# MarvelMathesh/sincformer-metacog-speech-enhancement

Hardware: AMD Instinct MI355X
Metric: audio frames/sec/GPU (16 kHz, 512-frame utts) + mask RMSE vs CPU ref (higher is better)
Workload: dtype fp16 MFMA operands (PerceptionAgent, fusion, Conformer GEMMs, heads) + bf16 attention core, fp32 accumulate (ops.POLICIES['mixed']); 1 GPU; B256 x 512-frame utterances (L40880, T512) forward; batch_per_gpu=256, samples=40880, frames_per_utt=512, launch=eager launches, streams=2, precision_policy=mixed

## Files before the change

include/sincformer_hip.h:

```cpp
#ifndef SINCFORMER_HIP_H
#define SINCFORMER_HIP_H
#ifdef __cplusplus
extern "C" {
#endif

#define SFM_OK 0
#define SFM_ERR_ARG (-1)
#define SFM_ERR_SHAPE (-2)
#define SFM_ERR_LAUNCH (-3)
#define SFM_DT_BF16 0
#define SFM_DT_F16 1

#define SFM_EPI_NONE 0
#define SFM_EPI_SWISH 1
#define SFM_EPI_GELU 2
#define SFM_EPI_RESID 3
#define SFM_EPI_GLU 4
#define SFM_EPI_SIGMOID 5
#define SFM_EPI_TANH_SCALE 6
#define SFM_EPI_SIGMA 7
#define SFM_EPI_CPEA 8

#define SFM_LAYERNORM_MAX_D 512
#define SFM_ATTN_QTILE 128
// ... 201 lines not shown
                      int act, int dtype, float* ws, void* stream);
long long sfm_gn_bwd_reduce_ws_floats(int B, int L, int C);
int sfm_gn_bwd_coefs(float* S, const float* gamma1, const float* rstd1, const float* gamma2, const float* rstd2,
                     float* coef1, float* coef2, float* dparam, int B, int L, int C, int G, void* stream);
int sfm_gn_bwd_apply(const void* dout, int dout_f32, const void* x1, int x1_f32, const float* sc1, const float* sh1,
                     const float* mean1, const float* rstd1, const float* coef1, void* dx1, int dx1_f32, const void* x2,
                     int x2_f32, const float* sc2, const float* sh2, const float* mean2, const float* rstd2,
                     const float* coef2, void* dx2, int dx2_f32, int B, int L, int C, int G, int act, int dtype,
                     void* stream);
int sfm_maa_update_stats(const float* sigma, long long n, double* acc, float* stats, long long* num_updates, float momentum,
                         void* stream);
int sfm_maa_forward(const float* sigma, const float* stats, const float* params, float* logits, float* probs,
                    long long* decisions, float* confidence, long long n, void* stream);
int sfm_maa_backward(const float* sigma, const float* stats, const float* params, const float* g_logits, const float* g_probs,
                     const float* g_conf, float* dsigma, void* H1, void* H2, void* dZ1, void* dZ2, void* GL, void* XN,
                     long long n, int dtype, void* stream);
int sfm_vq_forward(const float* x, const float* centroids, int M, float* q, long long* idx, double* acc, long long n,
                   void* stream);
int sfm_vq_backward(const float* x, const long long* idx, const float* centroids, int M, const float* g_q,
                    const float* g_loss, float beta, float* dx, float* dcent, long long n, void* stream);
long long sfm_sumsq_ws_doubles(long long n);
int sfm_sumsq(const float* g, long long n, double* out, double* ws, void* stream);
int sfm_adamw_step(float* p, float* g, float* m, float* v, long long n, double* ctl, float lr, float beta1, float beta2,
                   float eps, float wd, float inv_scale, float max_norm, int write_back_grad, void* stream);
int sfm_adamw_step_masked(float* p, float* g, float* m, float* v, long long n, double* ctl, float lr, float beta1, float beta2,
                          float eps, float wd, float inv_scale, float max_norm, int write_back_grad, const long long* spans,
                          const float* touched, int n_params, void* stream);
int sfm_adamw_step_scaled(float* p, float* g, float* m, float* v, long long n, double* ctl, float lr, float beta1, float beta2,
                          float eps, float wd, float inv_world, float max_norm, int write_back_grad, const long long* spans,
                          const float* touched, int n_params, float* loss_scale, float growth_factor, float backoff_factor,
                          int growth_interval, void* stream);
long long sfm_tn_ws_floats(int M, int N, int K);
int sfm_gemm16_tn(const void* G, const void* X, float* dW, float* db, int M, int N, int K, int ldg, int ldx, int ldw,
                  int dtype, float* ws, long long ws_floats, void* stream);
int sfm_conv_wgrad16(const void* G, const void* x, float* dW, float* db, int B, int Lout, int Lin, int Cin, int N, int ksize,
                     int stride, int pad, long long x_batch_stride, int ldg, int ldw, int dtype, float* ws, long long ws_floats,
                     void* stream);
long long sfm_colsum_ws_floats(int M, int N);
int sfm_colsum(const void* G, float* out, int M, int N, int ldg, int g_f32, int dtype, float* ws, void* stream);
long long sfm_layernorm_bwd_ws_floats(int M, int D);
int sfm_layernorm_bwd(const float* x, const float* gamma, const float* dy, const float* dres, float* dx,
                      float* dgamma, float* dbeta, int M, int D, int ldx, int ld, float eps, float* ws, void* stream);
int sfm_layernorm_bwd_ex(const float* x, const float* gamma, const void* dy, int dy_16, const float* dres, float* dx,
                         float* dgamma, float* dbeta, int M, int D, int ldx, int ldy, int ld, float eps, int dtype,
                         float* ws, void* stream);
int sfm_layernorm_bwd_next(const float* x, const float* gamma, const void* dy, int dy_16, const float* dres, float* dx,
                           float* dgamma, float* dbeta, int M, int D, int ldx, int ldy, int ld, float eps, int dtype,
                           void* next16, float next_alpha, float next_p, unsigned int next_seed, float* ws, void* stream);
int sfm_ew_train(const void* z, const void* g, void* out, long long M, int N, int mode, int g_f32, int out_f32,
                 float alpha, float p, unsigned int seed, int dtype, void* stream);
long long sfm_col_stats_ws_floats(int M, int C);
int sfm_col_stats(const float* y, const float* aux, const float* mean, const float* rstd, float* S, int M, int C, float* ws,
                  void* stream);
int sfm_col_pilot(const float* y, float* K, int M, int C, void* stream);
int sfm_col_stats_shifted(const float* y, const float* K, float* S, int M, int C, float* ws, void* stream);
int sfm_add_cols(const float* a, const float* b, float* out, long long M, int C, int Cb, long long lda, long long ldb, long long ldo,
                 void* stream);
int sfm_lstm_hprev16(const float* h, void* out, int B, int T, int H, int dtype, void* stream);
int sfm_bn_finalize(const float* S, const float* K, const float* gamma, const float* beta, float* run_mean, float* run_var,
                    float* mean, float* rstd, float* sc, float* sh, int C, long long M, float eps, float momentum, int eval_mode,
                    void* stream);
int sfm_bn_swish_bwd(const void* g, const float* y, const float* mean, const float* rstd, const float* gamma,
                     const float* beta, float* S, float* dy, int M, int C, int g_f32, int pass, int dtype,
                     float* ws, void* stream);
long long sfm_dwconv_wgrad_scratch_floats(int B, int T, int C, int KS);
int sfm_dwconv_wgrad(const void* x, const float* dy, float* dw, float* db, float* scratch, int B, int T, int C, int KS,
                     int dtype, void* stream);
int sfm_attention_fwd_train(const void* qkv, void* out, float* lse, int B, int T, int H, int hd, int ldqkv,
                            int ldo, int koff, int voff, long long qkv_batch_stride, long long o_batch_stride,
                            float scale, float p_drop, unsigned int seed, int dtype, void* stream);
int sfm_attention_bwd(const void* qkv, const void* O, const void* dO, const float* lse, float* delta, void* dqkv,
                      int B, int T, int H, int hd, int ldqkv, int ldo, int koff, int voff, float p_drop,
                      unsigned int seed, int dtype, void* stream);
int sfm_lin256(const void* A, const void* W, const float* bias, void* out, int M, int NW, int lda, int ldo, int glu, int dtype,
               int out_dtype, void* stream);
int sfm_ln_lin256(const float* X32, int ldx, const float* lnw, const float* lnb, float eps, const void* W, const float* bias,
                  void* out, int M, int NW, int ldo, int glu, int dtype, int out_dtype, void* stream);
int sfm_headpool_frames_per_tile(int Tin, int Tout);
int sfm_headpool(const void* xd, const void* W, const float* bias, void* pooled, float* gn_partial, int B, int Tin, int Tout, int NW,
                 int lda, int ldp, int gcols, int dtype, void* stream);

int sfm_bilstm_layer(const float* xg, const float* whh, float* out, int B, int T, int H, int dtype, void* stream);
int sfm_bilstm_layer_ex(const float* xg, const float* whh, float* out, int B, int T, int H, int w16, void* stream);
int sfm_bilstm_layer_train_ex(const float* xg, const float* whh, float* out, float* save, int B, int T, int H, int w16, void* stream);
int sfm_bilstm_layer_train(const float* xg, const float* whh, float* out, float* save, int B, int T, int H, int dtype,
                           void* stream);
int sfm_bilstm_layer_bwd(const float* save, const float* whh, const float* dout, float* dxg, int B, int T, int H,
                         void* stream);
int sfm_memory_fwd(const float* emb, const float* params, float* bias_out, float* gate_out, int* top_idx,
                   float* sim_out, int B, int key_dim, int value_dim, int slots, float temperature, void* stream);
long long sfm_memory_param_floats(int key_dim, int value_dim, int slots);
long long sfm_memory_bwd_ws_floats(int B, int key_dim, int value_dim, int slots);
int sfm_memory_bwd(const float* emb, const float* params, const float* d_out, const float* d_gate, float* d_emb,
                   float* dparams, int B, int key_dim, int value_dim, int slots, float temperature, float* ws, void* stream);

long long sfm_pstoi_loss_ws_doubles(int B, int T, int frame_len);
int sfm_pstoi_loss(const float* e0, const float* e1, const float* c0, const float* c1, const float* band_w, float* loss,
                   float* g0, float* g1, double* ws, int B, int T, int F, int NB, int frame_len, float beta_db, int layout,
                   void* stream);
long long sfm_mse_loss_ws_doubles(long long n);
int sfm_mse_loss(const float* pred, const float* target, float* loss, float* grad, double* ws, long long n, void* stream);

int sfm_adv_sn_fwd(const long long* table, int n_layers, void* packed, void* packed_lo, float* saved, int training, float eps,
                   int dtype, void* stream);
int sfm_adv_sn_bwd(const float* G, const float* W, const float* u, const float* v, const float* sigma, float* dW,
                   const float* db_in, float* db, const float* g, float cnorm, int N, int Cin, int ksize, int Cp, int accumulate,
                   void* stream);
int sfm_adv_stage(const float* x, const float* im, void* x16, void* x16lo, float* x32, int B, int F, int T, int Cp, int pair,
                  int dtype, void* stream);
int sfm_adv_stage_bwd(const float* d, const float* re, const float* im, float* dx, float* dx_im, const float* g, float cnorm, int B,
                      int F, int T, int Cp, int pair, void* stream);
long long sfm_adv_leaky_ws_doubles(long long n);
int sfm_adv_leaky(const float* z, const float* z_real, void* a16, void* a16lo, double* ws, double* loss, float scale, long long n,
                  int dtype, void* stream);
int sfm_adv_leaky_bwd(const float* incoming, const float* z, const float* z_real, const float* g, float w_fm, float cnorm,
                      void* dz16, long long n, int dtype, void* stream);
int sfm_adv_pool(const float* in32, float* out32, void* out16, void* out16lo, int B, int Tin, int F, int Cp, int dtype,
                 void* stream);
int sfm_adv_pool_bwd(const float* dnext, float* dx, int B, int Tin, int Cp, void* stream);
long long sfm_adv_head_ws_doubles(int B, int T);
int sfm_adv_head(const void* a16, const void* a16lo, const void* w16, const void* w16lo, const float* bias, float* out, double* ws,
                 double* loss, float target, float scale, int B, int T, int C, int dtype, void* stream);
long long sfm_adv_head_bwd_ws_floats(int B, int T, int C);
int sfm_adv_head_bwd(const void* a16, const void* w16, const float* out, const float* g, float coef, float cnorm, float target,
                     float* da, float* dwb, float* ws, int B, int T, int C, int dtype, void* stream);

int sfm_mask_irm(const float* clean_mag, const float* noise_mag, float* out, long long n, float p, float eps, void* stream);
int sfm_mask_corr(const float* noisy, const float* clean, const float* noise, float* rho_s, float* rho_n, long long n, float eps,
                  void* stream);
int sfm_mask_pcirm(const float* clean_mag, const float* noise_mag, const float* rho_s, const float* rho_n, const float* phi1,
                   const float* phi2, float* out, long long n, float eps, void* stream);
int sfm_mask_quantize(const float* pcirm, const double* table, float* out, long long n, int M, void* stream);
long long sfm_mix_scale_ws_doubles(int B, int L);
int sfm_mix_scale(const float* clean, const float* bank, const int* bank_off, const int* noise_ids, const float* snr_db,
                  const int* lengths, double* ws, float* scale, int B, int L, int n_noise, void* stream);
int sfm_mix_apply(const float* clean, const float* bank, const int* bank_off, const int* noise_ids, const int* lengths,
                  const float* scale, float* noisy, float* noise_rows, int B, int L, int n_noise, void* stream);
int sfm_curriculum_mask(const float* cr, const float* ci, const float* nr, const float* ni, const float* scale,
                        const double* table, float* yr, float* yi, float* mask, int B, int T, int F, int kind, float p, float eps,
                        int M, void* stream);

int sfm_pso_frame_coef(const float* pcirm, const double* table, double* a, double* b, int B, int C, int T, int M, void* stream);
long long sfm_pso_split_ws_doubles(int B, int Lmax);
int sfm_pso_split(const float* noisy, const float* clean, const int* lengths, const int* samp_off, const double* a,
                  const double* b, float* ya, float* yb, float* clean_packed, double* ws, double* S, int B, int Lmax, int T,
                  int frame, int hop, void* stream);
int sfm_pso_fitness(const float* cr, const float* ci, const float* ar, const float* ai, const float* br, const float* bi,
                    const int* frame_off, const int* lengths, const double* S, const double* pos, const int* stopped,
                    double* partial, int B, int N, int F, int NC, void* stream);
int sfm_pso_step(const double* partial, const double* fitness, const int* frame_off, const double* draws, const double* params,
                 double* pos, double* vel, double* pbest_pos, double* pbest_fit, double* gbest, double* hist, int* iters,
                 int* stopped, int B, int N, int NC, int it, int max_iter, int maximize, void* stream);
int sfm_pso_quantize(const float* pcirm, const double* table, const double* middle, float* out, int B, long long CT, int M,
                     void* stream);

int sfm_gammatone_fir(const float* sig, const float* taps, const int* lengths, float* out, int B, int L, int C, int K, void* stream);
int sfm_gammatone_tf_fits(int K, int hop);
int sfm_gammatone_tf(const float* sig, const float* taps, const float* tw, const int* lengths, float* partial, int B, int L, int C,
                     int K, int hop, int nblocks, void* stream);
int sfm_gammatone_moments(const float* y, const float* tw, const int* lengths, float* partial, int B, int L, int C, int T, int w,
                          int frame, int hop, void* stream);
int sfm_gammatone_tf_finish(const float* partial, const float* rot, const int* lengths, float* mag, float* phase, float* re,
                            float* im, int B, int C, int T, int P, int two, int L, int frame, int hop, int N, void* stream);

int sfm_haircell(const float* x, const double* par, double* out, int N, int L, void* stream);
int sfm_haircell_frames(const float* x, const double* par, const int* lengths, double* frames, int N, int C, int L, int frame,
// ... 31 lines not shown
```

sincformer_metacog_speech_enhancement_amd/csrc/lstm.hip:

```cpp
#include "sfm_common.h"

constexpr int LSTM_FWD_LPU = 4;

#define DPP_XOR1 0xB1
#define DPP_XOR2 0x4E
#define DPP_HALF_MIRROR 0x141
#define DPP_Q0 0x00
#define DPP_Q1 0x55
#define DPP_Q2 0xAA
#define DPP_Q3 0xFF

__device__ __forceinline__ float fast_sigmoid(float x) {
  return __builtin_amdgcn_rcpf(1.0f + __builtin_amdgcn_exp2f(-1.44269504088896340736f * x));
}

template <int H, int LPU>
__global__ __launch_bounds__(LPU * H) void bilstm_layer_kernel(const float* __restrict__ xg,
                                                               const float* __restrict__ whh,
                                                               float* __restrict__ out, int T, float* __restrict__ save) {
  constexpr int KS = H / LPU;
  constexpr int SL = KS + 4;
  __shared__ __attribute__((aligned(16))) float hs[2][LPU * SL];
  const int tid = threadIdx.x;
  const int j = tid / LPU, ks = tid % LPU;
  const int dir = blockIdx.x, b = blockIdx.y;
  float w[4][KS];
#pragma unroll
  for (int g = 0; g < 4; ++g) {
    const float* wr = whh + ((long long)dir * 4 * H + g * H + j) * H + ks * KS;
#pragma unroll
    for (int i = 0; i < KS; ++i) w[g][i] = wr[i];
  }
  if (tid < LPU * SL) { hs[0][tid] = 0.f; hs[1][tid] = 0.f; }
  __syncthreads();
  float c = 0.f;
  const int mygate = ks & 3;
  const float* xb = xg + (long long)b * T * (8 * H) + (long long)dir * 4 * H + mygate * H + j;
  float* ob = out + (long long)b * T * (2 * H) + dir * H + j;
  int t = dir ? (T - 1) : 0;
  const int dt = dir ? -1 : 1;
  const float gsc = (mygate == 2) ? 2.0f : 1.0f, gof = (mygate == 2) ? -1.0f : 0.0f;
  const int hslot = (j / KS) * SL + (j % KS);
  float xnext = xb[(long long)t * (8 * H)];
  for (int s = 0; s < T; ++s, t += dt) {
    const float xcur = xnext;
    if (s + 1 < T) xnext = xb[(long long)(t + dt) * (8 * H)];
    const float* hc = hs[s & 1] + ks * SL;
    float a[4] = {0.f, 0.f, 0.f, 0.f};
#pragma unroll
    for (int i = 0; i < KS; i += 4) {
      const f32x4 hv = *reinterpret_cast<const f32x4*>(hc + i);
#pragma unroll
      for (int g = 0; g < 4; ++g) {
        a[g] += w[g][i] * hv[0];
        a[g] += w[g][i + 1] * hv[1];
        a[g] += w[g][i + 2] * hv[2];
        a[g] += w[g][i + 3] * hv[3];
      }
    }
#pragma unroll
    for (int g = 0; g < 4; ++g) {
      a[g] = dpp_perm_add<DPP_XOR1>(a[g]);
      a[g] = dpp_perm_add<DPP_XOR2>(a[g]);
      if (LPU == 8) a[g] = dpp_perm_add<DPP_HALF_MIRROR>(a[g]);
    }
    const float pre = ((mygate == 0) ? a[0] : (mygate == 1) ? a[1] : (mygate == 2) ? a[2] : a[3]) + xcur;
    const float act = gsc * fast_sigmoid(gsc * pre) + gof;
    const float ig = dpp_perm<DPP_Q0>(act), fg = dpp_perm<DPP_Q1>(act);
    const float cg = dpp_perm<DPP_Q2>(act), og = dpp_perm<DPP_Q3>(act);
    c = fg * c + ig * cg;
    const float h = og * (2.0f * fast_sigmoid(2.0f * c) - 1.0f);
    if (ks == 0) {
      hs[(s + 1) & 1][hslot] = h;
      ob[(long long)t * (2 * H)] = h;
    }
    if (save) {
      float* sv = save + ((((long long)b * T + t) * 2 + dir) * 5) * H + j;
      if (ks < 4) sv[mygate * H] = act;
      if (ks == LPU - 4) sv[4 * H] = c;
    }
    asm volatile("s_waitcnt lgkmcnt(0)\n\ts_barrier" ::: "memory");
  }
}

typedef _Float16 lstm_h2 __attribute__((ext_vector_type(2)));
template <int H, int LPU, bool SAVE>
__global__ __launch_bounds__(LPU * H, 4) void bilstm_layer16_kernel(const float* __restrict__ xg, const float* __restrict__ whh,
                                                                    float* __restrict__ out, int T, float* __restrict__ save) {
  constexpr int KS = H / LPU;
  constexpr int KW = KS / 2;
  constexpr int SLW = KW + 4;
  static_assert(KW % 4 == 0, "16-byte slice reads");
  __shared__ __attribute__((aligned(16))) uint32_t hs[2][LPU * SLW];
  const int tid = threadIdx.x;
  const int j = tid / LPU, ks = tid % LPU;
  const int dir = blockIdx.x, b = blockIdx.y;
  lstm_h2 w[4][KW];
#pragma unroll
  for (int g = 0; g < 4; ++g) {
    const float* wr = whh + ((long long)dir * 4 * H + g * H + j) * H + ks * KS;
#pragma unroll
    for (int i = 0; i < KW; ++i) w[g][i] = lstm_h2{(_Float16)wr[2 * i], (_Float16)wr[2 * i + 1]};
    __builtin_amdgcn_sched_barrier(0);
  }
  if (tid < LPU * SLW) { hs[0][tid] = 0u; hs[1][tid] = 0u; }
  __syncthreads();
  float c = 0.f;
  const int mygate = ks & 3;
  const float* xb = xg + (long long)b * T * (8 * H) + (long long)dir * 4 * H + mygate * H + j;
  float* ob = out + (long long)b * T * (2 * H) + dir * H + j;
  int t = dir ? (T - 1) : 0;
  const int dt = dir ? -1 : 1;
  const float gsc = (mygate == 2) ? 2.0f : 1.0f, gof = (mygate == 2) ? -1.0f : 0.0f;
  const uint32_t hbase = (uint32_t)(uintptr_t)(lds_ptr_t)&hs[0][0];
  const uint32_t hslot = hbase + ((j / KS) * SLW * 2 + (j % KS)) * 2;
  const uint32_t hread = hbase + ks * SLW * 4;
  float xnext = xb[(long long)t * (8 * H)];
  for (int s = 0; s < T; ++s, t += dt) {
    const float xcur = xnext;
    if (s + 1 < T) xnext = xb[(long long)(t + dt) * (8 * H)];
    const uint32_t hc = hread + (uint32_t)((s & 1) * LPU * SLW * 4);
    float a[4] = {0.f, 0.f, 0.f, 0.f};
    u32x4 hv[KW / 4];
#pragma unroll
    for (int q = 0; q < KW / 4; ++q) asm volatile("ds_read_b128 %0, %1 offset:%2" : "=v"(hv[q]) : "v"(hc), "n"(q * 16) : "memory");
    if constexpr (KW / 4 == 4) {
      asm volatile("s_waitcnt lgkmcnt(2)" : "+v"(hv[0]), "+v"(hv[1])::"memory");
      asm volatile("s_waitcnt lgkmcnt(0)" : "+v"(hv[2]), "+v"(hv[3])::"memory");
    } else {
      static_assert(KW / 4 == 2, "H 128 or 64 with 4 lanes per unit");
      asm volatile("s_waitcnt lgkmcnt(0)" : "+v"(hv[0]), "+v"(hv[1])::"memory");
    }
#pragma unroll
    for (int q = 0; q < KW / 4; ++q) {
#pragma unroll
      for (int e = 0; e < 4; ++e) {
        const uint32_t hd = hv[q][e];
        const lstm_h2 hp = __builtin_bit_cast(lstm_h2, hd);
#pragma unroll
        for (int g = 0; g < 4; ++g) a[g] = __builtin_amdgcn_fdot2(w[g][4 * q + e], hp, a[g], false);
      }
    }
#pragma unroll
    for (int g = 0; g < 4; ++g) {
      a[g] = dpp_perm_add<DPP_XOR1>(a[g]);
      a[g] = dpp_perm_add<DPP_XOR2>(a[g]);
      if (LPU == 8) a[g] = dpp_perm_add<DPP_HALF_MIRROR>(a[g]);
    }
    const float pre = ((mygate == 0) ? a[0] : (mygate == 1) ? a[1] : (mygate == 2) ? a[2] : a[3]) + xcur;
    const float act = gsc * fast_sigmoid(gsc * pre) + gof;
    const float ig = dpp_perm<DPP_Q0>(act), fg = dpp_perm<DPP_Q1>(act);
    const float cg = dpp_perm<DPP_Q2>(act), og = dpp_perm<DPP_Q3>(act);
    c = fg * c + ig * cg;
    const float h = og * (2.0f * fast_sigmoid(2.0f * c) - 1.0f);
    if (ks == 0) {
      const uint32_t hb = (uint32_t)__builtin_bit_cast(unsigned short, (_Float16)h);
      asm volatile("ds_write_b16 %0, %1" ::"v"(hslot + (uint32_t)(((s + 1) & 1) * LPU * SLW * 4)), "v"(hb) : "memory");
      ob[(long long)t * (2 * H)] = h;
    }
    if (SAVE) {
      float* sv = save + ((((long long)b * T + t) * 2 + dir) * 5) * H + j;
      if (ks < 4) sv[mygate * H] = act;
      if (ks == LPU - 4) sv[4 * H] = c;
    }
    asm volatile("s_waitcnt lgkmcnt(0)\n\ts_barrier" ::: "memory");
  }
}

template <int H, int LPU>
__global__ __launch_bounds__(LPU * H) void bilstm_layer_bwd_kernel(const float* __restrict__ save,
                                                                 const float* __restrict__ whh,
                                                                 const float* __restrict__ dout,
                                                                 float* __restrict__ dxg, int T) {
  constexpr int G4 = 4 * H;
  constexpr int KS = G4 / LPU;
  constexpr int SL = KS + 4;
  __shared__ __attribute__((aligned(16))) float das[2][LPU * SL];
  const int tid = threadIdx.x;
  const int j = tid / LPU, ks = tid % LPU;
  const int dir = blockIdx.x, b = blockIdx.y;
  float w[KS];
#pragma unroll
  for (int i = 0; i < KS; ++i) w[i] = whh[((long long)dir * G4 + ks * KS + i) * H + j];
  for (int i = tid; i < LPU * SL; i += LPU * H) { das[0][i] = 0.f; das[1][i] = 0.f; }
  __syncthreads();
  const long long cb = (long long)b * T;
  float dh_rec = 0.f, dc_next = 0.f;
  const int dt = dir ? -1 : 1;
  int t = dir ? 0 : (T - 1);
  float nx[7] = {0.f, 0.f, 0.f, 0.f, 0.f, 0.f, 0.f};
  auto fetch = [&](int tt) {
    const float* sv = save + (((cb + tt) * 2 + dir) * 5) * H + j;
    nx[0] = sv[0]; nx[1] = sv[H]; nx[2] = sv[2 * H]; nx[3] = sv[3 * H]; nx[4] = sv[4 * H];
    const int tp = tt - dt;
    nx[5] = (tp >= 0 && tp < T) ? save[(((cb + tp) * 2 + dir) * 5 + 4) * H + j] : 0.f;
    nx[6] = dout[(cb + tt) * (2 * H) + dir * H + j];
  };
  if (ks == 0) fetch(t);
  for (int s = 0; s < T; ++s, t -= dt) {
    if (ks == 0) {
      const float ig = nx[0], fg = nx[1], gg = nx[2], og = nx[3], c = nx[4], cp = nx[5];
      const float dh = nx[6] + dh_rec;
      if (s + 1 < T) fetch(t - dt);
      const float tc = 2.0f * fast_sigmoid(2.0f * c) - 1.0f;
      const float dc = dh * og * (1.0f - tc * tc) + dc_next;
      const float dai = dc * gg * ig * (1.0f - ig);
      const float daf = dc * cp * fg * (1.0f - fg);
      const float dag = dc * ig * (1.0f - gg * gg);
      const float dao = dh * tc * og * (1.0f - og);
      dc_next = dc * fg;
      float* dx = dxg + (cb + t) * (8 * H) + (long long)dir * G4 + j;
      dx[0] = dai; dx[H] = daf; dx[2 * H] = dag; dx[3 * H] = dao;
      float* da = das[s & 1];
      da[((0 * H + j) / KS) * SL + (0 * H + j) % KS] = dai;
      da[((1 * H + j) / KS) * SL + (1 * H + j) % KS] = daf;
      da[((2 * H + j) / KS) * SL + (2 * H + j) % KS] = dag;
      da[((3 * H + j) / KS) * SL + (3 * H + j) % KS] = dao;
    }
    asm volatile("s_waitcnt lgkmcnt(0)\n\ts_barrier" ::: "memory");
    const float* dc_ = das[s & 1] + ks * SL;
    float a = 0.f, a2 = 0.f;
#pragma unroll
    for (int i = 0; i < KS; i += 8) {
      const f32x4 v = *reinterpret_cast<const f32x4*>(dc_ + i);
      const f32x4 u = *reinterpret_cast<const f32x4*>(dc_ + i + 4);
      a += w[i] * v[0];
      a2 += w[i + 4] * u[0];
      a += w[i + 1] * v[1];
      a2 += w[i + 5] * u[1];
      a += w[i + 2] * v[2];
      a2 += w[i + 6] * u[2];
      a += w[i + 3] * v[3];
      a2 += w[i + 7] * u[3];
    }
    a += a2;
    a = dpp_perm_add<DPP_XOR1>(a);
    a = dpp_perm_add<DPP_XOR2>(a);
    if (LPU == 8) a = dpp_perm_add<DPP_HALF_MIRROR>(a);
    dh_rec = a;
  }
}

template <int H>
static int bilstm_fwd_go(const float* xg, const float* whh, float* out, float* save, int B, int T, hipStream_t st, bool w16 = false) {
  constexpr int LPU = H >= 64 ? LSTM_FWD_LPU : 8;
  if constexpr (H >= 64 && (H / LPU) % 8 == 0) {
    if (w16) {
      if (save) SFM_LAUNCH((bilstm_layer16_kernel<H, LPU, true>), dim3(2, B), dim3(LPU * H), 0, st, xg, whh, out, T, save);
      else SFM_LAUNCH((bilstm_layer16_kernel<H, LPU, false>), dim3(2, B), dim3(LPU * H), 0, st, xg, whh, out, T, save);
      return SFM_OK;
    }
  }
  SFM_LAUNCH((bilstm_layer_kernel<H, LPU>), dim3(2, B), dim3(LPU * H), 0, st, xg, whh, out, T, save);
  return SFM_OK;
}

extern "C" int sfm_bilstm_layer_train(const float* xg, const float* whh, float* out, float* save, int B, int T, int H,
                                      int dtype, void* stream) {
  (void)dtype;
  if (!xg || !whh || !out) return SFM_ERR_ARG;
  if (B <= 0 || T <= 0) return SFM_ERR_SHAPE;
  hipStream_t st = (hipStream_t)stream;
  if (H == 128) return bilstm_fwd_go<128>(xg, whh, out, save, B, T, st);
  if (H == 64) return bilstm_fwd_go<64>(xg, whh, out, save, B, T, st);
  if (H == 32) return bilstm_fwd_go<32>(xg, whh, out, save, B, T, st);
  return SFM_ERR_SHAPE;
}

extern "C" int sfm_bilstm_layer(const float* xg, const float* whh, float* out, int B, int T, int H, int dtype,
                                void* stream) {
  return sfm_bilstm_layer_train(xg, whh, out, nullptr, B, T, H, dtype, stream);
}

extern "C" int sfm_bilstm_layer_train_ex(const float* xg, const float* whh, float* out, float* save, int B, int T, int H, int w16,
                                         void* stream) {
  if (!xg || !whh || !out || !save) return SFM_ERR_ARG;
  if (B <= 0 || T <= 0) return SFM_ERR_SHAPE;
  hipStream_t st = (hipStream_t)stream;
  if (H == 128) return bilstm_fwd_go<128>(xg, whh, out, save, B, T, st, w16 != 0);
  if (H == 64) return bilstm_fwd_go<64>(xg, whh, out, save, B, T, st, w16 != 0);
  if (H == 32) return bilstm_fwd_go<32>(xg, whh, out, save, B, T, st, false);
  return SFM_ERR_SHAPE;
}

extern "C" int sfm_bilstm_layer_ex(const float* xg, const float* whh, float* out, int B, int T, int H, int w16, void* stream) {
  if (!xg || !whh || !out) return SFM_ERR_ARG;
  if (B <= 0 || T <= 0) return SFM_ERR_SHAPE;
  hipStream_t st = (hipStream_t)stream;
  if (H == 128) return bilstm_fwd_go<128>(xg, whh, out, nullptr, B, T, st, w16 != 0);
  if (H == 64) return bilstm_fwd_go<64>(xg, whh, out, nullptr, B, T, st, w16 != 0);
  if (H == 32) return bilstm_fwd_go<32>(xg, whh, out, nullptr, B, T, st, false);
  return SFM_ERR_SHAPE;
}

extern "C" int sfm_bilstm_layer_bwd(const float* save, const float* whh, const float* dout, float* dxg, int B, int T, int H,
                                    void* stream) {
  if (!save || !whh || !dout || !dxg) return SFM_ERR_ARG;
  if (B <= 0 || T <= 0) return SFM_ERR_SHAPE;
  hipStream_t st = (hipStream_t)stream;
  static const int lpu = getenv("SFM_LSTM_BWD_LPU") ? atoi(getenv("SFM_LSTM_BWD_LPU")) : 4;
  if (H == 128 && lpu == 4) SFM_LAUNCH((bilstm_layer_bwd_kernel<128, 4>), dim3(2, B), dim3(512), 0, st, save, whh, dout, dxg, T);
  else if (H == 128) SFM_LAUNCH((bilstm_layer_bwd_kernel<128, 8>), dim3(2, B), dim3(1024), 0, st, save, whh, dout, dxg, T);
  else if (H == 64) SFM_LAUNCH((bilstm_layer_bwd_kernel<64, 8>), dim3(2, B), dim3(512), 0, st, save, whh, dout, dxg, T);
  else if (H == 32) SFM_LAUNCH((bilstm_layer_bwd_kernel<32, 8>), dim3(2, B), dim3(256), 0, st, save, whh, dout, dxg, T);
  else return SFM_ERR_SHAPE;
  return SFM_OK;
}
```

sincformer_metacog_speech_enhancement_amd/functional.py:

```python
import math
import numpy as np
import torch

from . import ops

N_FFT, HOP, WIN = 256, 80, 160
N_FREQ = N_FFT // 2 + 1
SINC_ON_16BIT_MFMA = True
FUSE_LD = 1088


def _f32(t):
    return t.detach().float().contiguous()


def sub(sd, prefix):
    p = prefix + "."
    return {k[len(p):]: v for k, v in sd.items() if k.startswith(p)}


def add_to16(x32, y32, C):
    M = x32.numel() // C
    dev = x32.device
    one = _const(dev, C, 1.0)
# ... 526 lines not shown
            r2, p2, P2, _, _, _ = _convp((r1, s1, h1), bp["c2"], B, L1, 1, 1, G, dt)
            s2, h2 = ops.gn_finalize(p2, bp["g2w"], bp["g2b"], B, P2, G, C, L1)
            inp = (r2, s2, h2, rs, ss, hs)
            Lc = L1
        rd, pd, Pd, Tpa, _, _ = _convp(inp, pk["down"], B, Lc, 2, 2, 16, dt)
    else:
        x = torch.empty(B, L, C0, device=dev, dtype=dt)
        ops.gn_apply(raw, sc, sh, x, B, L, C0, act=1)
        del raw
        for bp in pk["blocks"]:
            G, C = bp["groups"], bp["cout"]
            r1, p1, P1, L1 = _conv_gn(x, bp["c1"], B, Lc, 2, 3, G, dt)
            s1, h1 = ops.gn_finalize(p1, bp["g1w"], bp["g1b"], B, P1, G, C, L1)
            a1 = torch.empty(B, L1, C, device=dev, dtype=dt)
            ops.gn_apply(r1, s1, h1, a1, B, L1, C, act=1)
            r2, p2, P2, _ = _conv_gn(a1, bp["c2"], B, L1, 1, 1, G, dt)
            rs, ps, Ps, _ = _conv_gn(x, bp["cs"], B, Lc, 2, 0, G, dt)
            s2, h2 = ops.gn_finalize(p2, bp["g2w"], bp["g2b"], B, P2, G, C, L1)
            ss, hs = ops.gn_finalize(ps, bp["gsw"], bp["gsb"], B, Ps, G, C, L1)
            x = torch.empty(B, L1, C, device=dev, dtype=dt)
            ops.gn_apply(r2, s2, h2, x, B, L1, C, act=1, x2=rs, sc2=ss, sh2=hs)
            Lc = L1
        rd, pd, Pd, Tpa = _conv_gn(x, pk["down"], B, Lc, 2, 2, 16, dt)
    sd_, hd_ = ops.gn_finalize(pd, pk["dn_w"], pk["dn_b"], B, Pd, 16, D, Tpa)
    xd = torch.empty(B, Tpa, D, device=dev, dtype=dt)
    ops.gn_apply(rd, sd_, hd_, xd, B, Tpa, D, act=1)
    tiles = None
    if not latents and pool_to is not None and D == 256 and pk["zproj"].Npad == 2 * D and pk["zproj"].ksize == 1:
        tiles = ops.headpool_tiles(Tpa, pool_to)
    if tiles is not None:
        rz = torch.empty(B, pool_to, 2 * D, device=dev, dtype=dt)
        pz = torch.empty(B, tiles[1], 32, 2, device=dev, dtype=torch.float32)
        ops.headpool(xd, pk["zproj"], rz, pz, B, Tpa, pool_to, gcols=(2 * D) // 32)
        Pz = tiles[1]
    else:
        rz, pz, Pz, _ = _conv_gn(xd, pk["zproj"], B, Tpa, 1, 0, 32, torch.float32 if latents else dt)
    sz, hz = ops.gn_finalize(pz, pk["z_w"], pk["z_b"], B, Pz, 32, 2 * D, Tpa)
    if latents:
        zcat = torch.empty(B, Tpa, 2 * D, device=dev, dtype=torch.float32)
        ops.gn_apply(rz, sz, hz, zcat, B, Tpa, 2 * D, act=0)
    else:
        zcat = (rz, sz, hz)
    u = torch.empty(B, Tpa, pk["u0"].N, device=dev, dtype=dt)
    ops.gemm16(xd, pk["u0"], u, B=B, Lout=Tpa, Lin=Tpa, a_batch_stride=Tpa * D, ldo=pk["u0"].N,
               o_batch_stride=Tpa * pk["u0"].N, stride=1, pad=1, epi=ops.EPI_GELU)
    sigma = torch.empty(B * Tpa, 1, device=dev, dtype=torch.float32)
    ops.linear16(u.reshape(B * Tpa, -1), pk["u2"], epi=ops.EPI_SIGMA, out=sigma)
    return zcat, sigma.reshape(B, Tpa)


def pack_cpea(sd, num_layers=2):
    with ops.stage("front"):
        return _pack_cpea(sd, num_layers)


def _pack_cpea(sd, num_layers):
    pk = {"layers": [], "H": sd["lstm.weight_hh_l0"].shape[1]}
    for l in range(num_layers):
        wih = torch.cat([sd["lstm.weight_ih_l%d" % l], sd["lstm.weight_ih_l%d_reverse" % l]], dim=0)
        bias = torch.cat([sd["lstm.bias_ih_l%d" % l] + sd["lstm.bias_hh_l%d" % l],
                          sd["lstm.bias_ih_l%d_reverse" % l] + sd["lstm.bias_hh_l%d_reverse" % l]], dim=0)
        whh = torch.stack([_f32(sd["lstm.weight_hh_l%d" % l]), _f32(sd["lstm.weight_hh_l%d_reverse" % l])], dim=0)
        pk["layers"].append({"wih": ops.pack_linear(wih, bias), "whh": whh.contiguous()})
    wh = torch.cat([sd["rho_s_head.0.weight"], sd["rho_n_head.0.weight"], sd["phi1_head.0.weight"],
                    sd["phi2_head.0.weight"]], dim=0)
    bh = torch.cat([sd["rho_s_head.0.bias"], sd["rho_n_head.0.bias"], sd["phi1_head.0.bias"], sd["phi2_head.0.bias"]], dim=0)
    pk["heads"] = ops.pack_linear(wh, bh)
    pk["oc"] = sd["rho_s_head.0.weight"].shape[0]
    return pk


def cpea_forward(z16, pk, B, T, out=None):
    with ops.stage("front"):
        return _cpea_forward(z16, pk, B, T, out)


def _cpea_forward(z16, pk, B, T, out):
    H = pk["H"]
    M = B * T
    dt = ops.compute_dtype()
    x16 = z16
    for lp in pk["layers"]:
        xg = ops.linear16(x16, lp["wih"], out_dtype=torch.float32)
        h = ops.bilstm_layer(xg, lp["whh"], B, T, H, w16=ops.lstm_w16())
        x16 = torch.empty(M, 2 * H, device=h.device, dtype=dt)
        ops.convert_rows(h, x16, M, 2 * H, 2 * H, 2 * H, 2 * H)
    oc = pk["oc"]
    if out is None:
        out = torch.empty(M, 4 * oc, device=x16.device, dtype=torch.float32)
    ops.linear16(x16, pk["heads"], epi=ops.EPI_CPEA, alpha=math.pi, nsplit=2 * oc, out=out)
    return out


def pack_memory_params(sd):
    order = ["key_proj.0.weight", "key_proj.0.bias", "key_proj.1.weight", "key_proj.1.bias", "key_proj.3.weight",
             "key_proj.3.bias", "keys", "values", "value_proj.0.weight", "value_proj.0.bias", "gate.0.weight",
             "gate.0.bias"]
    return torch.cat([_f32(sd[k]).reshape(-1) for k in order]).contiguous()


def pack_msa(sd, num_blocks, num_heads=4):
    with ops.stage("front"):
        pk = {"f0": ops.pack_linear(sd["fusion.0.weight"], sd["fusion.0.bias"], k_pad_to=FUSE_LD),
              "f1w": _f32(sd["fusion.1.weight"]), "f1b": _f32(sd["fusion.1.bias"]),
              "f3": ops.pack_linear(sd["fusion.3.weight"], sd["fusion.3.bias"]),
              "f4w": _f32(sd["fusion.4.weight"]), "f4b": _f32(sd["fusion.4.bias"])}
    pk["conf"] = pack_complex_conformer(sub(sd, "conformer"), num_blocks, num_heads)
    with ops.stage("tail"):
        pk.update({"r0": ops.pack_linear(sd["mask_proj_real.0.weight"], sd["mask_proj_real.0.bias"]),
                   "r2": ops.pack_linear(sd["mask_proj_real.2.weight"], sd["mask_proj_real.2.bias"]),
                   "i0": ops.pack_linear(sd["mask_proj_imag.0.weight"], sd["mask_proj_imag.0.bias"]),
                   "i2": ops.pack_linear(sd["mask_proj_imag.2.weight"], sd["mask_proj_imag.2.bias"])})
    pk["d_model"] = sd["fusion.3.weight"].shape[0]
    return pk


def msa_logits(fused16, pk, B, T, H):
    D = pk["d_model"]
    with ops.stage("front"):
        h = ops.linear16(fused16, pk["f0"], out_dtype=torch.float32)
        h16 = _ln16(h, pk["f1w"], pk["f1b"], act=1)
        h = ops.linear16(h16, pk["f3"], out_dtype=torch.float32)
        hf16 = _ln16(h, pk["f4w"], pk["f4b"])
    y16 = complex_conformer_core(hf16, pk["conf"], B, T, H)
    half = D // 2
    with ops.stage("tail"):
        gr = ops.linear16(y16[:, :half], pk["r0"], epi=ops.EPI_GELU)
        lm = ops.linear16(gr, pk["r2"], out_dtype=torch.float32)
        gi = ops.linear16(y16[:, half:], pk["i0"], epi=ops.EPI_GELU)
        lp = ops.linear16(gi, pk["i2"], out_dtype=torch.float32)
    return lm, lp


def msa_pack_inputs(z_real, z_imag, cpea, noisy_real, noisy_imag):
    with ops.stage("front"):
        return _msa_pack_inputs(z_real, z_imag, cpea, noisy_real, noisy_imag)


def _msa_pack_inputs(z_real, z_imag, cpea, noisy_real, noisy_imag):
    B, D, T = z_real.shape
    M = B * T
    dev = z_real.device
    fused = torch.empty(M, FUSE_LD, device=dev, dtype=ops.compute_dtype())
    zr, zi = z_real.float().contiguous(), z_imag.float().contiguous()
    ops.transpose(zr, fused, B, D, T, D * T, T, T * FUSE_LD, FUSE_LD)
    ops.transpose(zi, fused[:, D:], B, D, T, D * T, T, T * FUSE_LD, FUSE_LD)
    col = 2 * D
    for k in ("rho_s", "rho_n", "phi1", "phi2"):
        c = cpea[k].float().contiguous()
        oc = c.shape[-1]
        ops.convert_rows(c, fused[:, col:], M, oc, oc, oc, FUSE_LD)
        col += oc
    nr, ni = noisy_real.float().contiguous(), noisy_imag.float().contiguous()
    F = nr.shape[-1]
    ops.stft_lognorm_pack(nr, ni, fused[:, col:], M, F, FUSE_LD - col - 2 * F, FUSE_LD)
    return fused, nr, ni


PHASE_SCALE_MSA = 3.14159 / 8.0


def msa_forward(z_real, z_imag, cpea, noisy_real, noisy_imag, pk, H, mag_bias=None):
    B, D, T = z_real.shape
    fused, nr, ni = msa_pack_inputs(z_real, z_imag, cpea, noisy_real, noisy_imag)
    lm, lp = msa_logits(fused, pk, B, T, H)
    F = nr.shape[-1]
# ... 83 lines not shown
```

sincformer_metacog_speech_enhancement_amd/ops.py:

```python
import ctypes
import math
import re as _re
import numpy as np
import torch

from . import lib as _lib

_K = _lib.CONSTANTS
EPI_NONE, EPI_SWISH, EPI_GELU, EPI_RESID, EPI_GLU, EPI_SIGMOID, EPI_TANH_SCALE, EPI_SIGMA, EPI_CPEA = (
    _K["EPI_" + _n] for _n in ("NONE", "SWISH", "GELU", "RESID", "GLU", "SIGMOID", "TANH_SCALE", "SIGMA", "CPEA"))

_DT_ID = {torch.bfloat16: _K["DT_BF16"], torch.float16: _K["DT_F16"]}
import os as _os
TRAIN_DTYPE = torch.float16
_state = {"dtype": TRAIN_DTYPE}

_SWITCHES = {
    "gemm_variant": ["SFM_GEMM_VARIANT", 0, 0],
    "attention_variant": [None, 0, 0],
    "lin256": ["SFM_LIN256", True, True],
    "headpool": ["SFM_HEADPOOL", True, True],
    "lstm_w16": ["SFM_LSTM_W16", True, True],
    "deterministic": ["SFM_DETERMINISTIC", True, True],
    "wgrad_stream": ["SFM_WGRAD_STREAM", True, True],
# ... 1679 lines not shown
    return out


def bn_finalize(S, K, gamma, beta, run_mean, run_var, M, eps, momentum, eval_mode=False):
    L = _lib.load()
    C = gamma.numel()
    buf = torch.empty(4, C, device=gamma.device, dtype=torch.float32)
    _call("col_stats", L.sfm_bn_finalize, (_p(S), _p(K), _p(gamma), _p(beta), _p(run_mean), _p(run_var), _p(buf[0]), _p(buf[1]),
                                           _p(buf[2]), _p(buf[3]), C, M, float(eps), float(momentum), 1 if eval_mode else 0,
                                           _stream()))
    return buf[0], buf[1], buf[2:3], buf[3:4]


def bn_swish_bwd(g, y32, mean, rstd, gamma, beta, eval_mode=False):
    L = _lib.load()
    M, C = y32.shape
    S = torch.zeros(C, 2, device=y32.device, dtype=torch.float32)
    dy = torch.empty_like(y32)
    gf = 1 if g.dtype == torch.float32 else 0
    ws = _ws(int(L.sfm_col_stats_ws_floats(M, C)), y32.device) if switch("deterministic") else None
    for ps in (0, 1):
        Sx = torch.zeros_like(S) if (eval_mode and ps == 1) else S
        _call("bn_swish_bwd", L.sfm_bn_swish_bwd, (_p(g), _p(y32), _p(mean), _p(rstd), _p(gamma), _p(beta), _p(Sx), _p(dy), M, C, gf,
                                                   ps, _dt(), _p(ws), _stream()))
    return dy, S[:, 1].contiguous(), S[:, 0].contiguous()


def dwconv_wgrad(x16, dy32, B, T, C, KS, dw=None, db=None):
    L = _lib.load()
    dw = torch.zeros(C, KS, device=x16.device, dtype=torch.float32) if dw is None else dw
    db = torch.zeros(C, device=x16.device, dtype=torch.float32) if db is None else db
    scratch = torch.empty(int(L.sfm_dwconv_wgrad_scratch_floats(B, T, C, KS)), device=x16.device, dtype=torch.float32)
    _call("dwconv_wgrad", L.sfm_dwconv_wgrad, (_p(x16), _p(dy32), _p(dw), _p(db), _p(scratch), B, T, C, KS, _dt(), _stream()))
    return dw, db


def attention_train(qkv16, B, T, H, hd, p_drop=0.0, seed=0):
    L = _lib.load()
    D = H * hd
    ld = qkv16.stride(0)
    out = torch.empty(B * T, D, device=qkv16.device, dtype=qkv16.dtype)
    lse = torch.empty(B, H, T, device=qkv16.device, dtype=torch.float32)
    _call("attention_fwd", L.sfm_attention_fwd_train, (_p(qkv16), _p(out), _p(lse), B, T, H, hd, ld, out.stride(0), D, 2 * D,
                                                       T * ld, T * out.stride(0), -1.0, float(p_drop), int(seed) & 0xffffffff,
                                                       _dt(), _stream()), 4.0 * B * H * T * T * hd, 4.0 * B * T * D * 2)
    return out, lse


def attention_bwd(qkv16, O16, dO16, lse, B, T, H, hd, p_drop=0.0, seed=0):
    L = _lib.load()
    D = H * hd
    dqkv = torch.empty_like(qkv16)
    if hd != 64:
        scratch = torch.zeros(B * T, 2 * D, device=qkv16.device, dtype=torch.float32)
        _call("attention_bwd", L.sfm_attention_bwd_generic, (_p(qkv16), _p(O16), _p(dO16), _p(lse), _p(scratch), _p(dqkv), B, T, H,
                                                             hd, qkv16.stride(0), O16.stride(0), D, 2 * D, float(p_drop),
                                                             int(seed) & 0xffffffff, _dt(), _stream()),
              10.0 * B * H * T * T * hd, 8.0 * B * T * D * 2)
        return dqkv
    delta = torch.empty(B, H, T, device=qkv16.device, dtype=torch.float32)
    _call("attention_bwd", L.sfm_attention_bwd, (_p(qkv16), _p(O16), _p(dO16), _p(lse), _p(delta), _p(dqkv), B, T, H, hd,
                                                 qkv16.stride(0), O16.stride(0), D, 2 * D, float(p_drop), int(seed) & 0xffffffff,
                                                 _dt(), _stream()), 10.0 * B * H * T * T * hd, 8.0 * B * T * D * 2)
    return dqkv


def set_lstm_w16(flag):
    _SWITCHES["lstm_w16"][2] = bool(flag)


def lstm_w16():
    return switch("lstm_w16")


def bilstm_layer(xg, whh, B, T, H, w16=False):
    L = _lib.load()
    out = torch.empty(B, T, 2 * H, device=xg.device, dtype=torch.float32)
    flops, nbytes = 2.0 * B * T * 2 * 4 * H * H, B * T * (8 * H + 2 * H) * 4
    if w16:
        _call("bilstm_layer", L.sfm_bilstm_layer_ex, (_p(xg), _p(whh), _p(out), B, T, H, 1, _stream()), flops, nbytes)
    else:
        _call("bilstm_layer", L.sfm_bilstm_layer, (_p(xg), _p(whh), _p(out), B, T, H, _dt(), _stream()), flops, nbytes)
    return out


def bilstm_layer_train(xg, whh, B, T, H, w16=None):
    L = _lib.load()
    out = torch.empty(B, T, 2 * H, device=xg.device, dtype=torch.float32)
    save = torch.empty(B, T, 2, 5, H, device=xg.device, dtype=torch.float32)
    if w16 is None:
        w16 = switch("lstm_w16") and _state["dtype"] == torch.float16
    if w16:
        _call("bilstm_layer", L.sfm_bilstm_layer_train_ex, (_p(xg), _p(whh), _p(out), _p(save), B, T, H, 1, _stream()))
    else:
        _call("bilstm_layer", L.sfm_bilstm_layer_train, (_p(xg), _p(whh), _p(out), _p(save), B, T, H, _dt(), _stream()))
    return out, save


def bilstm_layer_bwd(save, whh, dout, B, T, H):
    L = _lib.load()
    dxg = torch.empty(B, T, 2, 4 * H, device=dout.device, dtype=torch.float32)
    _call("bilstm_bwd", L.sfm_bilstm_layer_bwd, (_p(save), _p(whh), _p(dout), _p(dxg), B, T, H, _stream()))
    return dxg


def stft_lognorm_bwd(re, im, g, M, F):
    L = _lib.load()
    dre, dim_ = torch.empty_like(re), torch.empty_like(im)
    _call("stft_lognorm_bwd", L.sfm_stft_lognorm_bwd, (_p(re), _p(im), _p(g), _p(dre), _p(dim_), M, F, g.stride(0), _stream()))
    return dre, dim_


def memory_bwd(emb, params, d_out, d_gate, key_dim, value_dim, slots, temperature, want_d_emb=True):
    L = _lib.load()
    Bn = emb.shape[0]
    d_emb = torch.empty(Bn, key_dim, device=emb.device, dtype=torch.float32) if want_d_emb else None
    dparams = torch.zeros_like(params)
    ws = None
    if switch("deterministic"):
        npar = int(L.sfm_memory_param_floats(key_dim, value_dim, slots))
        if npar != params.numel():
            raise RuntimeError("memory_bwd: the parameter blob has %d floats, the kernel's layout %d" % (params.numel(), npar))
        ws = _ws(L.sfm_memory_bwd_ws_floats(Bn, key_dim, value_dim, slots), emb.device)
    _call("memory_bwd", L.sfm_memory_bwd, (_p(emb), _p(params), _p(d_out), _p(d_gate), _p(d_emb), _p(dparams), Bn, key_dim, value_dim,
                                           slots, float(temperature), _p(ws), _stream()))
    return d_emb, dparams


def memory_fwd(emb, params, key_dim, value_dim, slots, temperature):
    L = _lib.load()
    Bn = emb.shape[0]
    dev = emb.device
    bias = torch.empty(Bn, value_dim, device=dev, dtype=torch.float32)
    gate = torch.empty(Bn, 1, device=dev, dtype=torch.float32)
    top = torch.empty(Bn, device=dev, dtype=torch.int32)
    sim = torch.empty(Bn, device=dev, dtype=torch.float32)
    _call("memory_fwd", L.sfm_memory_fwd, (_p(emb), _p(params), _p(bias), _p(gate), _p(top), _p(sim), Bn, key_dim, value_dim, slots,
                          float(temperature), _stream()))
    return bias, gate, top, sim


def _hann(n):
    k = np.arange(n, dtype=np.float64)
    return 0.5 - 0.5 * np.cos(2.0 * np.pi * k / n)


def stft_matrix(n_fft, win, device):
    F = n_fft // 2 + 1
    woff = (n_fft - win) // 2
    w = _hann(win)
    n = (np.arange(win, dtype=np.float64) + woff)[:, None]
    f = np.arange(F, dtype=np.float64)[None, :]
    ang = 2.0 * np.pi * ((n * f) % n_fft) / n_fft
    M = np.concatenate([w[:, None] * np.cos(ang), -w[:, None] * np.sin(ang)], axis=1)
    return pack_f32_matrix(torch.from_numpy(M.astype(np.float32)).to(device))


def istft_matrix(n_fft, win, device):
    F = n_fft // 2 + 1
    woff = (n_fft - win) // 2
    w = _hann(win)
    n = (np.arange(win, dtype=np.float64) + woff)[None, :]
    f = np.arange(F, dtype=np.float64)[:, None]
    ang = 2.0 * np.pi * ((f * n) % n_fft) / n_fft
    coef = np.full((F, 1), 2.0)
    coef[0, 0] = 1.0
# ... 439 lines not shown
```

Before: 8.508 million STFT frames/s (whole job).

## Use MFMA-based BiLSTM recurrence batching four chains and writing fp16 rows directly

Adds a new BiLSTM forward kernel for H=128 that packs four batch chains per block and computes the recurrent h·Whh product with 4x4x4 fp16 MFMA instructions instead of per-lane dot products. It prefetches input gate projections several steps ahead and double-buffers h in LDS. The inference path now writes fp16/bf16 output rows directly, removing the separate fp32 output buffer and convert_rows launch. This reduces block count and scalar FMA work on the serial recurrence, at the cost of fp16 weights and a fixed H=128 specialization.

```diff
diff --git a/include/sincformer_hip.h b/include/sincformer_hip.h
--- a/include/sincformer_hip.h
+++ b/include/sincformer_hip.h
@@ -307,6 +307,8 @@
 
 int sfm_bilstm_layer(const float* xg, const float* whh, float* out, int B, int T, int H, int dtype, void* stream);
 int sfm_bilstm_layer_ex(const float* xg, const float* whh, float* out, int B, int T, int H, int w16, void* stream);
+int sfm_bilstm_layer_rows16(const float* xg, const float* whh, void* out16, long long ld16, int B, int T, int H, int w16,
+                            int dtype, void* stream);
 int sfm_bilstm_layer_train_ex(const float* xg, const float* whh, float* out, float* save, int B, int T, int H, int w16, void* stream);
 int sfm_bilstm_layer_train(const float* xg, const float* whh, float* out, float* save, int B, int T, int H, int dtype,
                            void* stream);
diff --git a/sincformer_metacog_speech_enhancement_amd/csrc/lstm.hip b/sincformer_metacog_speech_enhancement_amd/csrc/lstm.hip
--- a/sincformer_metacog_speech_enhancement_amd/csrc/lstm.hip
+++ b/sincformer_metacog_speech_enhancement_amd/csrc/lstm.hip
@@ -1,4 +1,5 @@
 #include "sfm_common.h"
+#include <type_traits>
 
 constexpr int LSTM_FWD_LPU = 4;
 
@@ -165,6 +166,109 @@
     }
     asm volatile("s_waitcnt lgkmcnt(0)\n\ts_barrier" ::: "memory");
   }
+}
+
+typedef _Float16 lstm_h4 __attribute__((ext_vector_type(4)));
+constexpr int LSTM_MFMA_CHAINS = 4;
+constexpr int LSTM_OUT_F32 = -1;
+template <int OUT>
+__global__ __launch_bounds__(512) void bilstm_layer16_mfma_kernel(const float* __restrict__ xg, const float* __restrict__ whh,
+                                                                  void* __restrict__ out, long long ldo, int B, int T) {
+  typedef typename std::conditional<OUT == LSTM_OUT_F32, float, u16>::type out_t;
+  constexpr int H = 128;
+  constexpr int CS = 2 * H + 64;
+  constexpr int BUF = LSTM_MFMA_CHAINS * CS;
+  __shared__ __attribute__((aligned(16))) uint32_t hs[2 * BUF / 4];
+  const int tid = threadIdx.x;
+  const int u = tid >> 2, j = tid & 3;
+  const int dir = blockIdx.x;
+  const int chain = blockIdx.y * LSTM_MFMA_CHAINS + j;
+  const bool live = chain < B;
+  const int b = live ? chain : B - 1;
+  lstm_h4 w[H / 4];
+  {
+    const float* wr = whh + ((long long)dir * 4 * H + j * H + u) * H;
+#pragma unroll
+    for (int q = 0; q < 4; ++q) {
+#pragma unroll
+      for (int i = 0; i < 8; ++i) {
+        const f32x4 v = *reinterpret_cast<const f32x4*>(wr + 32 * q + 4 * i);
+        w[8 * q + i] = lstm_h4{(_Float16)v[0], (_Float16)v[1], (_Float16)v[2], (_Float16)v[3]};
+      }
+      __builtin_amdgcn_sched_barrier(0);
+    }
+  }
+  for (int i = tid; i < 2 * BUF / 4; i += 512) hs[i] = 0u;
+  __syncthreads();
+  float c = 0.f;
+  const int t0 = dir ? (T - 1) : 0, dt = dir ? -1 : 1;
+  const float* xb = xg + (((long long)b * T + t0) * 2 + dir) * (4 * H) + u;
+  out_t* ob = reinterpret_cast<out_t*>(out) + ((long long)b * T + t0) * ldo + dir * H + u;
+  const long long xstep = (long long)dt * (8 * H), ostep = (long long)dt * ldo;
+  const uint32_t hbase = (uint32_t)(uintptr_t)(lds_ptr_t)&hs[0];
+  const int grp = (tid >> 4) & 3;
+  const uint32_t hread = hbase + j * CS + grp * 16;
+  const uint32_t hslot = hbase + j * CS + u * 2;
+  constexpr int PF = 4;
+  f32x4 xr[PF];
+  auto fetch = [&](f32x4& x, int s) {
+    const float* xs = xb + (s < T ? s : T - 1) * xstep;
+#pragma unroll
+    for (int g = 0; g < 4; ++g) x[g] = xs[g * H];
+  };
+#pragma unroll
+  for (int i = 0; i < PF; ++i) fetch(xr[i], i);
+  auto step = [&](f32x4& x, int s, int par) {
+    f32x4 a0 = x, a1 = {0.f, 0.f, 0.f, 0.f}, a2 = a1, a3 = a1;
+    fetch(x, s + PF);
+    const uint32_t hc = hread + (uint32_t)(par * BUF);
+    u32x4 hv[4];
+#pragma unroll
+    for (int q = 0; q < 4; ++q) asm volatile("ds_read_b128 %0, %1 offset:%2" : "=v"(hv[q]) : "v"(hc), "n"(q * 64) : "memory");
+#define LSTM_MFMA_PAIR(q, g, acc0, acc1)                                                                                         \
+    acc0 = __builtin_amdgcn_mfma_f32_4x4x4f16(w[8 * q + 2 * g], __builtin_shufflevector(p, p, 0, 1, 2, 3), acc0, 0, 0, 4 + g);   \
+    acc1 = __builtin_amdgcn_mfma_f32_4x4x4f16(w[8 * q + 2 * g + 1], __builtin_shufflevector(p, p, 4, 5, 6, 7), acc1, 0, 0, 4 + g);
+#define LSTM_MFMA_GROUP(q, left)                                                                                                 \
+    {                                                                                                                            \
+      asm volatile("s_waitcnt lgkmcnt(" #left ")" : "+v"(hv[q])::"memory");                                                      \
+      const f16x8_t p = __builtin_bit_cast(f16x8_t, hv[q]);                                                                      \
+      LSTM_MFMA_PAIR(q, 0, a0, a1)                                                                                               \
+      LSTM_MFMA_PAIR(q, 1, a2, a3)                                                                                               \
+      LSTM_MFMA_PAIR(q, 2, a0, a1)                                                                                               \
+      LSTM_MFMA_PAIR(q, 3, a2, a3)                                                                                               \
+    }                                                                                                                            \
+    __builtin_amdgcn_sched_barrier(0);
+    LSTM_MFMA_GROUP(0, 3)
+    LSTM_MFMA_GROUP(1, 2)
+    LSTM_MFMA_GROUP(2, 1)
+    LSTM_MFMA_GROUP(3, 0)
+#undef LSTM_MFMA_GROUP
+#undef LSTM_MFMA_PAIR
+    const f32x4 pre = (a0 + a1) + (a2 + a3);
+    const float ig = fast_sigmoid(pre[0]), fg = fast_sigmoid(pre[1]);
+    const float cg = 2.0f * fast_sigmoid(2.0f * pre[2]) - 1.0f, og = fast_sigmoid(pre[3]);
+    c = fg * c + ig * cg;
+    float h = og * (2.0f * fast_sigmoid(2.0f * c) - 1.0f);
+    asm volatile("" : "+v"(h));
+    const uint32_t hb = (uint32_t)__builtin_bit_cast(unsigned short, (_Float16)h);
+    asm volatile("ds_write_b16 %0, %1" ::"v"(hslot + (uint32_t)((par ^ 1) * BUF)), "v"(hb) : "memory");
+    if (live) {
+      if constexpr (OUT == LSTM_OUT_F32) ob[s * ostep] = h;
+      else if constexpr (OUT == SFM_DT_F16) ob[s * ostep] = (u16)hb;
+      else ob[s * ostep] = BF16::from_f32(h);
+    }
+    asm volatile("s_waitcnt lgkmcnt(0)\n\ts_barrier" ::: "memory");
+  };
+  int s0 = 0;
+  for (; s0 + PF <= T; s0 += PF) {
+    step(xr[0], s0, 0);
+    step(xr[1], s0 + 1, 1);
+    step(xr[2], s0 + 2, 0);
+    step(xr[3], s0 + 3, 1);
+  }
+  if (s0 < T) step(xr[0], s0, 0);
+  if (s0 + 1 < T) step(xr[1], s0 + 1, 1);
+  if (s0 + 2 < T) step(xr[2], s0 + 2, 0);
 }
 
 template <int H, int LPU>
@@ -247,6 +351,9 @@
   if constexpr (H >= 64 && (H / LPU) % 8 == 0) {
     if (w16) {
       if (save) SFM_LAUNCH((bilstm_layer16_kernel<H, LPU, true>), dim3(2, B), dim3(LPU * H), 0, st, xg, whh, out, T, save);
+      else if constexpr (H == 128)
+        SFM_LAUNCH((bilstm_layer16_mfma_kernel<LSTM_OUT_F32>), dim3(2, (B + LSTM_MFMA_CHAINS - 1) / LSTM_MFMA_CHAINS), dim3(512), 0, st, xg,
+                   whh, (void*)out, (long long)(2 * H), B, T);
       else SFM_LAUNCH((bilstm_layer16_kernel<H, LPU, false>), dim3(2, B), dim3(LPU * H), 0, st, xg, whh, out, T, save);
       return SFM_OK;
     }
@@ -291,6 +398,17 @@
   if (H == 64) return bilstm_fwd_go<64>(xg, whh, out, nullptr, B, T, st, w16 != 0);
   if (H == 32) return bilstm_fwd_go<32>(xg, whh, out, nullptr, B, T, st, false);
   return SFM_ERR_SHAPE;
+}
+
+extern "C" int sfm_bilstm_layer_rows16(const float* xg, const float* whh, void* out16, long long ld16, int B, int T, int H, int w16,
+                                       int dtype, void* stream) {
+  if (!xg || !whh || !out16 || (dtype != SFM_DT_F16 && dtype != SFM_DT_BF16)) return SFM_ERR_ARG;
+  if (B <= 0 || T <= 0 || H != 128 || !w16 || ld16 < 2 * H) return SFM_ERR_SHAPE;
+  hipStream_t st = (hipStream_t)stream;
+  const dim3 grid(2, (B + LSTM_MFMA_CHAINS - 1) / LSTM_MFMA_CHAINS);
+  if (dtype == SFM_DT_F16) SFM_LAUNCH((bilstm_layer16_mfma_kernel<SFM_DT_F16>), grid, dim3(512), 0, st, xg, whh, out16, ld16, B, T);
+  else SFM_LAUNCH((bilstm_layer16_mfma_kernel<SFM_DT_BF16>), grid, dim3(512), 0, st, xg, whh, out16, ld16, B, T);
+  return SFM_OK;
 }
 
 extern "C" int sfm_bilstm_layer_bwd(const float* save, const float* whh, const float* dout, float* dxg, int B, int T, int H,
diff --git a/sincformer_metacog_speech_enhancement_amd/functional.py b/sincformer_metacog_speech_enhancement_amd/functional.py
--- a/sincformer_metacog_speech_enhancement_amd/functional.py
+++ b/sincformer_metacog_speech_enhancement_amd/functional.py
@@ -632,6 +632,9 @@
     x16 = z16
     for lp in pk["layers"]:
         xg = ops.linear16(x16, lp["wih"], out_dtype=torch.float32)
+        if H == 128 and ops.lstm_w16():
+            x16 = ops.bilstm_layer_rows16(xg, lp["whh"], B, T, H)
+            continue
         h = ops.bilstm_layer(xg, lp["whh"], B, T, H, w16=ops.lstm_w16())
         x16 = torch.empty(M, 2 * H, device=h.device, dtype=dt)
         ops.convert_rows(h, x16, M, 2 * H, 2 * H, 2 * H, 2 * H)
diff --git a/sincformer_metacog_speech_enhancement_amd/ops.py b/sincformer_metacog_speech_enhancement_amd/ops.py
--- a/sincformer_metacog_speech_enhancement_amd/ops.py
+++ b/sincformer_metacog_speech_enhancement_amd/ops.py
@@ -1785,6 +1785,16 @@
     else:
         _call("bilstm_layer", L.sfm_bilstm_layer, (_p(xg), _p(whh), _p(out), B, T, H, _dt(), _stream()), flops, nbytes)
     return out
+
+
+def bilstm_layer_rows16(xg, whh, B, T, H, out16=None):
+    L = _lib.load()
+    if out16 is None:
+        out16 = torch.empty(B * T, 2 * H, device=xg.device, dtype=compute_dtype())
+    flops, nbytes = 2.0 * B * T * 2 * 4 * H * H, B * T * (8 * H * 4 + 2 * H * 2)
+    _call("bilstm_layer", L.sfm_bilstm_layer_rows16, (_p(xg), _p(whh), _p(out16), out16.stride(0), B, T, H, 1, _dt(), _stream()),
+          flops, nbytes)
+    return out16
 
 
 def bilstm_layer_train(xg, whh, B, T, H, w16=None):
```

Result: faster. 8.918 million STFT frames/s (whole job) (median of 6 runs) (+4.8%).
